# Chanuk-Yang/Deep_Continuous_Fusion_for_Multi-Sensor_3D_Object_Detection

Hardware: AMD Instinct MI355X
Metric: frames/sec (train step) 100k-pt LiDAR + 1242x375 RGB (higher is better)
Workload: dtype bf16; 1 GPU; cfg2: grid 32x704x800, 100000 pts/frame, 1242x375 RGB, ResNet-18 image stream, K=3 fusion x4 sites, eval-mode BN (reference F4), batch 2/GPU; global_batch=2, parallelism=dp1, loss_sampling=compat, conv_chain=False

## Files before the change

### deep_continuous_fusion_for_multi-sensor_3d_object_detection_amd/csrc/geometry.hip

```cpp
#include <stdlib.h>
#include "dcf_common.h"
#include "proj_pred.h"

namespace {

struct Aff6 { float v[6]; };

constexpr int CP_THREADS = 256;
constexpr int CP_ITEMS = 4;
constexpr int CP_TILE = CP_THREADS * CP_ITEMS;

__device__ __forceinline__ int block_excl_scan(int v, int *total)
{
    __shared__ int wsum[4];
    const int lane = threadIdx.x & 63, wid = threadIdx.x >> 6;
    int inc = v;
#pragma unroll
    for (int o = 1; o < 64; o <<= 1) {
        int t = __shfl_up(inc, o, 64);
        if (lane >= o) inc += t;
    }
    if (lane == 63) wsum[wid] = inc;
    __syncthreads();
    int base = 0, tot = 0;
// ... 943 lines not shown
                const int t = t0 + lane;
                int a = 0, b = 0;
                if (R > 0) {
                    if (t < 2 * R + 1) { a = -R; b = -R + t; }
                    else if (t < 4 * R + 2) { a = R; b = -R + (t - (2 * R + 1)); }
                    else if (t < 6 * R + 1) { b = -R; a = -R + 1 + (t - (4 * R + 2)); }
                    else { b = R; a = -R + 1 + (t - (6 * R + 1)); }
                }
                const int bi = I + a, bj = J + b;
                int ps = 0, pe = 0;
                if (t < nblk && bi >= 0 && bi < g.h8 && bj >= 0 && bj < g.w8) {
                    const int k0 = (bi * g.w8 + bj) << 6;
                    ps = cellstart[k0];
                    pe = cellstart[k0 + 64];
                }
                unsigned long long live = __ballot(pe > ps);
                while (live) {
                    const int l = __ffsll((long long)live) - 1;
                    live &= live - 1;
                    const int cbi = __builtin_amdgcn_readlane(bi, l), cbj = __builtin_amdgcn_readlane(bj, l);
                    const int cps = __builtin_amdgcn_readlane(ps, l), cpe = __builtin_amdgcn_readlane(pe, l);
                    bool visit = true;
                    if (gcnt >= K) {
                        const float lox = ((float)(cbi * 8) * s - g.xo) / g.xs, hix = ((float)(cbi * 8 + 8) * s - g.xo) / g.xs;
                        const float loy = ((float)(cbj * 8) * s - g.yo) / g.ys, hiy = ((float)(cbj * 8 + 8) * s - g.yo) / g.ys;
                        const float ddx = fmaxf(0.f, fmaxf(lox - X, X - hix) - 1e-3f);
                        const float ddy = fmaxf(0.f, fmaxf(loy - Y, Y - hiy) - 1e-3f);
                        visit = (ddx * ddx + ddy * ddy) <= gd[K - 1];
                    }
                    if (visit) scan_range(cps, cpe);
                }
            }
            wave_merge<K>(top, gd, gi, gcnt);
            const float bound = (8.0f * (float)R + 0.5f) * cwmin - 1e-3f;
            if (gcnt >= K && gd[K - 1] < bound * bound) done = true;
            if (rmax2 >= 0.0f && bound > 0.f && bound * bound > rmax2) done = true;
        }
    }
    if (lane == 0) {
#pragma unroll
        for (int q = 0; q < K; ++q) out[q * hw + pix] = (q < gcnt) ? gi[q] : -1;
    }
}

template <int K>
__global__ void __launch_bounds__(256) k_knn_search_wave(const int *count, int n_max, KnnGrid g, const int *cellstart,
                                                         const float4 *sorted, float rmax2, int *out)
{
    knn_search_wave<K>(count, n_max, g, cellstart, sorted, rmax2, out, blockIdx.x);
}

constexpr int KNN_FINE_MIN_POINTS = 192;

__device__ __forceinline__ float open_edge_distance(const KnnGrid &gf, float X, float Y, int i0, int i1, int j0, int j1)
{
    const float s = (float)gf.stride;
    float b = 3.0e38f;
    if (i0 > 0) b = fminf(b, X - ((float)i0 * s - gf.xo) / gf.xs);
    if (i1 < gf.h - 1) b = fminf(b, ((float)(i1 + 1) * s - gf.xo) / gf.xs - X);
    if (j0 > 0) b = fminf(b, Y - ((float)j0 * s - gf.yo) / gf.ys);
    if (j1 < gf.w - 1) b = fminf(b, ((float)(j1 + 1) * s - gf.yo) / gf.ys - Y);
    return b - 1e-3f;
}

template <int K>
__device__ __forceinline__ void knn_search_fine(const int *count, int n_max, const KnnGrid &g, const KnnGrid &gf, const int *cellstart_c,
                                                const float4 *sorted_c, const int *cellstart, const float4 *sorted, float rmax2,
                                                int *out, int dense_min, const int bx)
{
    count += blockIdx.y * g.fs_cnt; out += (size_t)blockIdx.y * g.fs_out;
    cellstart_c += (size_t)blockIdx.y * g.fs_ws;
    sorted_c = reinterpret_cast<const float4 *>(reinterpret_cast<const int *>(sorted_c) + (size_t)blockIdx.y * g.fs_ws);
    cellstart += (size_t)blockIdx.y * gf.fs_ws;
    sorted = reinterpret_cast<const float4 *>(reinterpret_cast<const int *>(sorted) + (size_t)blockIdx.y * gf.fs_ws);
    const int lane = threadIdx.x & 63;
    const int pix = __builtin_amdgcn_readfirstlane(bx * 4 + (threadIdx.x >> 6));
    const int hw = g.h * g.w;
    if (pix >= hw) return;
    const int i = pix / g.w, j = pix - i * g.w;
    const float s = (float)g.stride;
    const float X = __fdiv_rn(__fsub_rn(__fmul_rn((float)i + 0.5f, s), g.xo), g.xs);
    const float Y = __fdiv_rn(__fsub_rn(__fmul_rn((float)j + 0.5f, s), g.yo), g.ys);
    const int n = min(*count, n_max);
    int ci, cj;
    point_cell(X, Y, gf, ci, cj);

    TopK<K> top;
    top.clear();
    float gd[K];
    int gi[K];
    int gcnt = 0;
#pragma unroll
    for (int q = 0; q < K; ++q) { gd[q] = 3.0e38f; gi[q] = 0x7fffffff; }
    auto scan_own = [&](int b, int e) {
        for (int p = b; p < e; ++p) {
            const float4 q = sorted[p];
            const float dx = __fsub_rn(q.x, X), dy = __fsub_rn(q.y, Y);
            const float d2 = __fadd_rn(__fmul_rn(dx, dx), __fmul_rn(dy, dy));
            if (!(rmax2 >= 0.0f && d2 > rmax2)) top.insert(d2, __float_as_int(q.z));
        }
    };
    auto scan_range = [&](int b, int e) {
        for (int p = b + lane; p < e; p += 64) {
            const float4 q = sorted_c[p];
            const float dx = __fsub_rn(q.x, X), dy = __fsub_rn(q.y, Y);
            const float d2 = __fadd_rn(__fmul_rn(dx, dx), __fmul_rn(dy, dy));
            if (!(rmax2 >= 0.0f && d2 > rmax2)) top.insert(d2, __float_as_int(q.z));
        }
    };
    bool done = (n == 0);
    bool dense = false;
    if (!done) {
        const int H8 = g.h8 * 8, W8 = g.w8 * 8;
        const int row = lane >> 1, part = lane & 1;
        const int wi = i - 2 + row;
        const int cbeg = max(j - 2, 0), cend = min(j + 2, W8 - 1);
        const int split = min(cend, (cbeg | 7));
        const int c0 = part == 0 ? cbeg : split + 1;
        const int c1 = part == 0 ? split : cend;
        int ps = 0, pe = 0;
        if (lane < 10 && wi >= 0 && wi <= H8 - 1 && c0 <= c1) {
            ps = cellstart_c[cell_key(wi, c0, g)];
            pe = cellstart_c[cell_key(wi, c1, g) + 1];
        }
        const int total = wave_sum_i(pe - ps);
        dense = total > dense_min;
        if (!dense) {
            unsigned long long live = __ballot(pe > ps);
            while (live) {
                const int l = __ffsll((long long)live) - 1;
                live &= live - 1;
                scan_range(__builtin_amdgcn_readlane(ps, l), __builtin_amdgcn_readlane(pe, l));
            }
            wave_merge<K>(top, gd, gi, gcnt);
            const float cw = fminf(s / g.xs, s / g.ys);
            const float bound = 2.5f * cw - 1e-3f;
            if (gcnt >= K && gd[K - 1] < bound * bound) done = true;
            if (rmax2 >= 0.0f && bound > 0.f && bound * bound > rmax2) done = true;
        }
    }
    int rprev = -1;
    for (int r = 2; r <= 8 && !done && dense; r += 2) {
        const int side = 2 * r + 1, ncell = side * side;
        for (int t0 = 0; t0 < ncell; t0 += 64) {
            const int t = t0 + lane;
            const int a = t / side - r, b = t - (t / side) * side - r;
            const int fi = ci + a, fj = cj + b;
            if (t < ncell && max(abs(a), abs(b)) > rprev && fi >= 0 && fi < gf.h && fj >= 0 && fj < gf.w) {
                const int key = cell_key(fi, fj, gf);
                scan_own(cellstart[key], cellstart[key + 1]);
            }
        }
        rprev = r;
        wave_merge<K>(top, gd, gi, gcnt);
        const float bound = open_edge_distance(gf, X, Y, ci - r, ci + r, cj - r, cj + r);
        if (gcnt >= K && bound > 0.f && gd[K - 1] < bound * bound) done = true;
        if (rmax2 >= 0.0f && bound > 0.f && bound * bound > rmax2) done = true;
    }
    if (!done) {
        top.clear();
        gcnt = 0;
#pragma unroll
        for (int q = 0; q < K; ++q) { gd[q] = 3.0e38f; gi[q] = 0x7fffffff; }
        const float cwmin = fminf(s / g.xs, s / g.ys);
        const int I = i >> 3, J = j >> 3;
        const int Rmax = max(g.h8, g.w8);
        for (int R = 0; R <= Rmax && !done; ++R) {
            const int nblk = R == 0 ? 1 : 8 * R;
            for (int t0 = 0; t0 < nblk; t0 += 64) {
                const int t = t0 + lane;
                int a = 0, b = 0;
                if (R > 0) {
                    if (t < 2 * R + 1) { a = -R; b = -R + t; }
                    else if (t < 4 * R + 2) { a = R; b = -R + (t - (2 * R + 1)); }
                    else if (t < 6 * R + 1) { b = -R; a = -R + 1 + (t - (4 * R + 2)); }
                    else { b = R; a = -R + 1 + (t - (6 * R + 1)); }
                }
                const int bi = I + a, bj = J + b;
                int ps = 0, pe = 0;
                if (t < nblk && bi >= 0 && bi < g.h8 && bj >= 0 && bj < g.w8) {
                    const int k0 = (bi * g.w8 + bj) << 6;
                    ps = cellstart_c[k0];
                    pe = cellstart_c[k0 + 64];
                }
                unsigned long long live = __ballot(pe > ps);
                while (live) {
                    const int l = __ffsll((long long)live) - 1;
                    live &= live - 1;
                    const int cbi = __builtin_amdgcn_readlane(bi, l), cbj = __builtin_amdgcn_readlane(bj, l);
                    const int cps = __builtin_amdgcn_readlane(ps, l), cpe = __builtin_amdgcn_readlane(pe, l);
                    bool visit = true;
                    if (gcnt >= K) {
                        const float lox = ((float)(cbi * 8) * s - g.xo) / g.xs, hix = ((float)(cbi * 8 + 8) * s - g.xo) / g.xs;
                        const float loy = ((float)(cbj * 8) * s - g.yo) / g.ys, hiy = ((float)(cbj * 8 + 8) * s - g.yo) / g.ys;
                        const float ddx = fmaxf(0.f, fmaxf(lox - X, X - hix) - 1e-3f);
                        const float ddy = fmaxf(0.f, fmaxf(loy - Y, Y - hiy) - 1e-3f);
                        visit = (ddx * ddx + ddy * ddy) <= gd[K - 1];
                    }
                    if (visit) scan_range(cps, cpe);
                }
            }
            wave_merge<K>(top, gd, gi, gcnt);
            const float bound = (8.0f * (float)R + 0.5f) * cwmin - 1e-3f;
            if (gcnt >= K && gd[K - 1] < bound * bound) done = true;
            if (rmax2 >= 0.0f && bound > 0.f && bound * bound > rmax2) done = true;
        }
    }
    if (lane == 0) {
#pragma unroll
        for (int q = 0; q < K; ++q) out[q * hw + pix] = (q < gcnt) ? gi[q] : -1;
    }
}

template <int K>
__global__ void __launch_bounds__(256) k_knn_search_fine(const int *count, int n_max, KnnGrid g, KnnGrid gf, const int *cellstart_c,
                                                         const float4 *sorted_c, const int *cellstart, const float4 *sorted, float rmax2,
                                                         int *out, int dense_min)
{
    knn_search_fine<K>(count, n_max, g, gf, cellstart_c, sorted_c, cellstart, sorted, rmax2, out, dense_min, blockIdx.x);
}

struct KnnSearchSites {
    KnnGrid g[DCF_MAX_KNN_SITES], gf[DCF_MAX_KNN_SITES];
    const int *cellstart[DCF_MAX_KNN_SITES], *cellstart_f[DCF_MAX_KNN_SITES];
    const float4 *sorted[DCF_MAX_KNN_SITES], *sorted_f[DCF_MAX_KNN_SITES];
    int *out[DCF_MAX_KNN_SITES];
    int kind[DCF_MAX_KNN_SITES];
    int first[DCF_MAX_KNN_SITES + 1];
    int n, dense_min;
};

template <int K>
__global__ void __launch_bounds__(256) k_knn_search_ms(const int *count, int n_max, KnnSearchSites S, float rmax2)
{
    int i = 0;
#pragma unroll
    for (int k = 1; k < DCF_MAX_KNN_SITES; ++k) i += (k < S.n && (int)blockIdx.x >= S.first[k]);
    const int lb = (int)blockIdx.x - S.first[i];
    const int wave = __builtin_amdgcn_readfirstlane(threadIdx.x >> 6);
    const KnnGrid &g = S.g[i];
    const int kind = S.kind[i];
    if (kind == 0) {
        const int tile = lb * 4 + wave;
        if (tile >= g.h8 * g.w8) return;
        knn_search_tile<K, 1>(count, n_max, g, S.cellstart[i], S.sorted[i], rmax2, S.out[i], tile, 0);
    } else if (kind == 1) {
        knn_search_tile<K, 4>(count, n_max, g, S.cellstart[i], S.sorted[i], rmax2, S.out[i], lb, wave);
    } else if (kind == 2) {
        knn_search_wave<K>(count, n_max, g, S.cellstart[i], S.sorted[i], rmax2, S.out[i], lb);
    } else {
        knn_search_fine<K>(count, n_max, g, S.gf[i], S.cellstart[i], S.sorted[i], S.cellstart_f[i], S.sorted_f[i], rmax2, S.out[i], S.dense_min, lb);
    }
}

struct InvMaps {
    const int *idx[DCF_MAX_KNN_MAPS];
    int first[DCF_MAX_KNN_MAPS + 1];
    int hw[DCF_MAX_KNN_MAPS], w[DCF_MAX_KNN_MAPS];
    int n;
};

__device__ __forceinline__ int inv_map_of(const InvMaps &m, int e)
{
    int g = 0;
#pragma unroll
    for (int i = 1; i < DCF_MAX_KNN_MAPS; ++i) g += (i < m.n && e >= m.first[i]);
    return g;
}

struct InvRun { int head, len; };
__device__ __forceinline__ InvRun inv_run(int key, int lane)
{
    const int prev = __shfl_up(key, 1, 64);
    const unsigned long long heads = __ballot(lane == 0 || key != prev);
    const unsigned long long below = heads & ((2ull << lane) - 1ull);
    InvRun r;
    r.head = 63 - __clzll(below);
    const unsigned long long above = lane == 63 ? 0ull : (heads >> (lane + 1));
    r.len = (above ? lane + 1 + (__ffsll((long long)above) - 1) : 64) - r.head;
    return r;
}

__global__ void __launch_bounds__(256) k_zero_rows(int *p, int n, int64_t stride)
{
    int4 *row = reinterpret_cast<int4 *>(p + blockIdx.y * stride);
    const int n4 = n >> 2;
    for (int i = blockIdx.x * blockDim.x + threadIdx.x; i < n4; i += gridDim.x * blockDim.x) row[i] = make_int4(0, 0, 0, 0);
    if (blockIdx.x == 0 && threadIdx.x < (n & 3)) p[blockIdx.y * stride + (n4 << 2) + threadIdx.x] = 0;
}

__device__ __forceinline__ int inv_load(const InvMaps &m, int e, int &g)
{
    const int e0 = blockIdx.x * blockDim.x;
    const int gA = __builtin_amdgcn_readfirstlane(inv_map_of(m, e0));
    const int gB = __builtin_amdgcn_readfirstlane(inv_map_of(m, min(e0 + (int)blockDim.x, m.first[m.n]) - 1));
    if (gA == gB) {
        g = gA;
        return m.idx[gA][e - m.first[gA]];
    }
    g = inv_map_of(m, e);
    return m.idx[g][e - m.first[g]];
}

__global__ void __launch_bounds__(256) k_inv_hist(InvMaps m, int n_max, int *cnt)
{
    const int e = blockIdx.x * blockDim.x + threadIdx.x;
    const int lane = threadIdx.x & 63;
    int key = -1;
    if (e < m.first[m.n]) {
        int g;
        const int id = inv_load(m, e, g);
        if (id >= 0 && id < n_max) key = g * (n_max + 1) + id;
    }
    const InvRun r = inv_run(key, lane);
    if (key >= 0 && r.head == lane) atomicAdd(&cnt[key], r.len);
}

__global__ void __launch_bounds__(256) k_inv_fill(InvMaps m, int n_max, int *cursor, int *ent_pix, int *ent_pt)
{
    const int e = blockIdx.x * blockDim.x + threadIdx.x;
    const int lane = threadIdx.x & 63;
    int key = -1, g = 0, id = 0;
    if (e < m.first[m.n]) {
        id = inv_load(m, e, g);
        if (id >= 0 && id < n_max) key = g * (n_max + 1) + id;
    }
    const InvRun r = inv_run(key, lane);
    int base = 0;
    if (key >= 0 && r.head == lane) base = atomicAdd(&cursor[key], r.len);
    base = __shfl(base, r.head, 64);
    if (key < 0) return;
    const int pos = base + (lane - r.head);
    const int p = (e - m.first[g]) % m.hw[g];
    ent_pix[pos] = ((p / m.w[g]) << 16) | (p % m.w[g]);
    ent_pt[pos] = id;
}

}

extern "C" size_t dcf_compact_workspace_bytes(int n) { return sizeof(int) * (size_t)(cdiv(n > 0 ? n : 1, CP_TILE) + 8); }

extern "C" int dcf_range_filter(const float *pts, int n, const float *lim, float *out_pts, int32_t *out_src,
                                int32_t *count_dev, void *ws, dcf_stream_t stream)
{
    DCF_REQUIRE(n >= 0 && lim && count_dev && ws, "dcf_range_filter: bad arguments");
    hipStream_t s = S(stream);
    if (n == 0) { DCF_HIP(hipMemsetAsync(count_dev, 0, sizeof(int), s)); return DCF_OK; }
    RangePred p;
    memcpy(p.lim.v, lim, sizeof(p.lim.v));
    int nb = cdiv(n, CP_TILE);
    int *bs = (int *)ws;
    DCF_LAUNCH_B("compact_count", (double)n * 12.0, s, hipLaunchKernelGGL(k_compact_count<RangePred>, dim3(nb), dim3(CP_THREADS), 0, s, pts, n, p, bs));
    DCF_LAUNCH("compact_scan", s, hipLaunchKernelGGL(k_compact_scan, dim3(1), dim3(CP_THREADS), 0, s, bs, nb, count_dev));
    DCF_LAUNCH_B("compact_scatter", (double)n * (12.0 + 16.0), s, hipLaunchKernelGGL((k_compact_scatter<RangePred, false>), dim3(nb), dim3(CP_THREADS), 0, s, pts, n, p, bs,
                                                         (float *)nullptr, out_pts, out_src));
    return DCF_OK;
}

extern "C" int dcf_project_filter(const float *pts, int n, const float *lim, const float *crt, float ulim, float vlim,
                                  int mode, float *uv_out, float *xyz_out, int32_t *src_out, int32_t *count_dev,
                                  void *ws, dcf_stream_t stream)
{
    DCF_REQUIRE(n >= 0 && lim && crt && count_dev && ws && uv_out && xyz_out, "dcf_project_filter: bad arguments");
    hipStream_t s = S(stream);
    if (n == 0) { DCF_HIP(hipMemsetAsync(count_dev, 0, sizeof(int), s)); return DCF_OK; }
    ProjPred p;
    memcpy(p.lim.v, lim, sizeof(p.lim.v));
    memcpy(p.c.v, crt, sizeof(p.c.v));
    p.ulim = ulim; p.vlim = vlim; p.mode = mode;
    int nb = cdiv(n, CP_TILE);
    int *bs = (int *)ws;
    DCF_LAUNCH_B("project_count", (double)n * 12.0, s, hipLaunchKernelGGL(k_compact_count<ProjPred>, dim3(nb), dim3(CP_THREADS), 0, s, pts, n, p, bs));
    DCF_LAUNCH("compact_scan", s, hipLaunchKernelGGL(k_compact_scan, dim3(1), dim3(CP_THREADS), 0, s, bs, nb, count_dev));
    DCF_LAUNCH_B("project_scatter", (double)n * (12.0 + 20.0), s, hipLaunchKernelGGL((k_compact_scatter<ProjPred, true>), dim3(nb), dim3(CP_THREADS), 0, s, pts, n, p, bs,
                                                         uv_out, xyz_out, src_out));
    return DCF_OK;
}

extern "C" int dcf_project_filter_batch(const float *const *pts, const int *n, int B, const float *lim, const float *crt, float ulim, float vlim,
                                        int mode, float *uv_out, float *xyz_out, int rows, int32_t *count_dev, void *ws, dcf_stream_t stream)
{
    const char *who = "dcf_project_filter_batch";
    DCF_REQUIRE(pts && n && lim && crt && count_dev && ws && uv_out && xyz_out, "%s: bad arguments", who);
    DCF_REQUIRE(B >= 1 && B <= DCF_PROJ_BATCH_MAX, "%s: 1..%d frames per call", who, DCF_PROJ_BATCH_MAX);
    hipStream_t s = S(stream);
    ProjBatch pb;
    int nmax = 0;
    for (int b = 0; b < DCF_PROJ_BATCH_MAX; ++b) {
        pb.pts[b] = b < B ? pts[b] : nullptr;
        pb.n[b] = b < B ? n[b] : 0;
        DCF_REQUIRE(b >= B || (n[b] >= 0 && n[b] <= rows && (n[b] == 0 || pts[b])), "%s: frame %d: bad point count / null points", who, b);
        memcpy(pb.c[b].v, crt + 12 * (b < B ? b : 0), sizeof(pb.c[b].v));
        if (b < B && n[b] > nmax) nmax = n[b];
    }
    if (nmax == 0) { DCF_HIP(hipMemsetAsync(count_dev, 0, sizeof(int) * B, s)); return DCF_OK; }
    Lim6 l;
    memcpy(l.v, lim, sizeof(l.v));
    const int nb = cdiv(nmax, CP_TILE);
    const int bstride = (int)(dcf_compact_workspace_bytes(nmax) / sizeof(int));
    int *bs = (int *)ws;
    DCF_LAUNCH_B("project_count", (double)nmax * B * 12.0, s, hipLaunchKernelGGL(k_proj_count_b, dim3(nb, B), dim3(CP_THREADS), 0, s, pb, l, ulim, vlim, mode, bs, bstride));
    DCF_LAUNCH("compact_scan", s, hipLaunchKernelGGL(k_proj_scan_b, dim3(1, B), dim3(CP_THREADS), 0, s, bs, nb, bstride, count_dev));
    DCF_LAUNCH_B("project_scatter", (double)nmax * B * (12.0 + 20.0), s, hipLaunchKernelGGL(k_proj_scatter_b, dim3(nb, B), dim3(CP_THREADS), 0, s, pb, l, ulim, vlim, mode, bs, bstride,
                                                                                    uv_out, xyz_out, rows));
    return DCF_OK;
}

extern "C" int dcf_augment_points_batch(const float *const *pts, const int *n, int B, const float *mat, const uint64_t *drop_key,
                                        const uint32_t *drop_thresh, float *const *out, dcf_stream_t stream)
{
    const char *who = "dcf_augment_points_batch";
    DCF_REQUIRE(pts && n && mat && drop_key && drop_thresh && out, "%s: bad arguments", who);
    DCF_REQUIRE(B >= 1 && B <= DCF_PROJ_BATCH_MAX, "%s: 1..%d frames per call", who, DCF_PROJ_BATCH_MAX);
    AugBatch ab;
    int nmax = 0;
    double total = 0.0;
    for (int b = 0; b < DCF_PROJ_BATCH_MAX; ++b) {
        const bool live = b < B;
        DCF_REQUIRE(!live || (n[b] >= 0 && (n[b] == 0 || (pts[b] && out[b]))), "%s: frame %d: bad point count / null points", who, b);
        DCF_REQUIRE(!live || ((((uintptr_t)pts[b]) | ((uintptr_t)out[b])) & 3) == 0, "%s: frame %d: pointers must be 4-byte aligned", who, b);
        ab.pts[b] = live ? pts[b] : nullptr;
        ab.out[b] = live ? out[b] : nullptr;
        ab.key[b] = live ? drop_key[b] : 0;
        ab.n[b] = live ? n[b] : 0;
        ab.thr[b] = live ? drop_thresh[b] : 0;
        for (int k = 0; k < 5; ++k) ab.m[b][k] = live ? mat[5 * b + k] : 0.f;
        if (live && n[b] > nmax) nmax = n[b];
        if (live) total += n[b];
    }
    for (int b = 0; b < B; ++b)
        for (int c = 0; c < B; ++c) {
            if (!n[b] || !n[c]) continue;
            const uintptr_t o0 = (uintptr_t)out[b], o1 = o0 + 12 * (uintptr_t)n[b];
            const uintptr_t p0 = (uintptr_t)pts[c], p1 = p0 + 12 * (uintptr_t)n[c];
            const uintptr_t q0 = (uintptr_t)out[c], q1 = q0 + 12 * (uintptr_t)n[c];
            DCF_REQUIRE((b == c && o0 == p0) || o1 <= p0 || p1 <= o0, "%s: output of frame %d overlaps the input of frame %d", who, b, c);
            DCF_REQUIRE(b == c || o1 <= q0 || q1 <= o0, "%s: outputs of frames %d and %d overlap", who, b, c);
        }
    if (nmax == 0) return DCF_OK;
    hipStream_t s = S(stream);
    DCF_LAUNCH_B("augment_points", total * 24.0, s, hipLaunchKernelGGL(k_augment_points_b, dim3(cdiv(nmax, AUG_TILE), B), dim3(AUG_THREADS), 0, s, ab));
    return DCF_OK;
}

extern "C" size_t dcf_voxelize_workspace_bytes(int Cz, int L, int W) { return sizeof(int) * 2 * (size_t)Cz * L * W; }

static bool voxel_cells_inside(const float *lim, const float *aff, int Cz, int L, int W, int64_t *lo_flat, int64_t *hi_flat)
{
    int64_t lo[3], hi[3];
    for (int ax = 0; ax < 3; ++ax) {
        const float p0 = nextafterf(lim[2 * ax], INFINITY), p1 = nextafterf(lim[2 * ax + 1], -INFINITY);
        if (!(p0 <= p1)) { *lo_flat = *hi_flat = 0; return true; }
        const float t0 = p0 * aff[2 * ax], t1 = p1 * aff[2 * ax];
        const float f0 = t0 + aff[2 * ax + 1], f1 = t1 + aff[2 * ax + 1];
        if (!(fabsf(f0) < 1073741824.0f && fabsf(f1) < 1073741824.0f)) return false;
        const int64_t c0 = (int64_t)(int)f0, c1 = (int64_t)(int)f1;
        lo[ax] = c0 < c1 ? c0 : c1;
        hi[ax] = c0 < c1 ? c1 : c0;
    }
    *lo_flat = (lo[2] * L + lo[0]) * W + lo[1];
    *hi_flat = (hi[2] * L + hi[0]) * W + hi[1];
    return *lo_flat >= 0 && *hi_flat < (int64_t)Cz * L * W;
}

static int voxel_guard(const char *who, const float *lim, const float *aff, int Cz, int L, int W)
{
    for (int k = 0; k < 6; ++k)
        DCF_REQUIRE(fabsf(lim[k]) <= 3.402823466e38f && fabsf(aff[k]) <= 3.402823466e38f, "%s: lim and aff must be finite", who);
    int64_t lo = 0, hi = 0;
    DCF_REQUIRE(voxel_cells_inside(lim, aff, Cz, L, W, &lo, &hi),
                "%s: a point inside the limits can fall into a cell outside the grid (flat cell index %lld .. %lld of %lld voxels)", who,
                (long long)lo, (long long)hi, (long long)Cz * L * W);
    return DCF_OK;
}


extern "C" int dcf_voxelize(const float *pts, int n, const float *lim, const float *aff, int Cz, int L, int W,
                            int mode, float *grid, void *owner_ws, dcf_stream_t stream)
{
    DCF_REQUIRE(n >= 0 && lim && aff && grid && Cz > 0 && L > 0 && W > 0, "dcf_voxelize: bad arguments");
    DCF_REQUIRE((int64_t)Cz * L * W < (1ll << 31), "dcf_voxelize: grid too large for int32 voxel ids");
    if (int rc = voxel_guard("dcf_voxelize", lim, aff, Cz, L, W)) return rc;
    hipStream_t s = S(stream);
    const int nvox = Cz * L * W;
    DCF_HIP(hipMemsetAsync(grid, 0, sizeof(float) * (size_t)nvox, s));
    if (n == 0) return DCF_OK;
    Lim6 l; Aff6 a;
    memcpy(l.v, lim, sizeof(l.v));
    memcpy(a.v, aff, sizeof(a.v));
    const int nb = cdiv(n, 256);
    if (mode == DCF_VOXEL_COMPAT) {
        DCF_REQUIRE(owner_ws != nullptr, "dcf_voxelize: compat mode needs the zeroed owner workspace");
        VoxBatch vb;
        for (int b = 0; b < DCF_MAX_VOXEL_BATCH; ++b) { vb.pts[b] = b == 0 ? pts : nullptr; vb.n[b] = b == 0 ? n : 0; }
        const dim3 g1(nb, 1);
        DCF_LAUNCH("voxel_cell_claim", s, hipLaunchKernelGGL(k_voxel_cell_claim, g1, dim3(256), 0, s, vb, l, a, L, W, nvox, (int *)owner_ws, 0));
        DCF_LAUNCH("voxel_cell_gather", s, hipLaunchKernelGGL((k_voxel_cell_gather<float, false>), g1, dim3(256), 0, s, vb, l, a, Cz, L, W, nvox, grid, (const int *)owner_ws));
        DCF_LAUNCH("voxel_cell_claim", s, hipLaunchKernelGGL(k_voxel_cell_claim, g1, dim3(256), 0, s, vb, l, a, L, W, nvox, (int *)owner_ws, 1));
    } else if (mode == DCF_VOXEL_COMPAT_ROUNDS) {
        DCF_REQUIRE(owner_ws != nullptr, "dcf_voxelize: compat mode needs the zeroed owner workspace");
        for (int r = 0; r <= 8; ++r)
            DCF_LAUNCH("voxel_compat_round", s, hipLaunchKernelGGL(k_voxel_compat_round, dim3(nb), dim3(256), 0, s, pts, n, l, a, L, W, nvox, r,
                                                                   grid, (int *)owner_ws));
    } else if (mode == DCF_VOXEL_ACCUM) {
        DCF_LAUNCH("voxel_accum", s, hipLaunchKernelGGL(k_voxel_accum, dim3(nb), dim3(256), 0, s, pts, n, l, a, L, W, nvox, grid));
    } else if (mode == DCF_VOXEL_OCCUPANCY) {
        DCF_LAUNCH("voxel_occupancy", s, hipLaunchKernelGGL(k_voxel_occupancy, dim3(nb), dim3(256), 0, s, pts, n, l, a, L, W, nvox, grid));
    } else {
        dcf_set_error("dcf_voxelize: unknown mode %d", mode);
        return DCF_EINVAL;
    }
    return DCF_OK;
}

static int voxelize_batch_impl(const char *who, int dtype, bool nhwc, const float *const *pts, const int *n, int B, const float *lim, const float *aff,
                               int Cz, int L, int W, void *grids, void *owner_ws, hipStream_t s)
{
    DCF_REQUIRE(pts && n && lim && aff && grids && owner_ws && Cz > 0 && L > 0 && W > 0, "%s: bad arguments", who);
    DCF_REQUIRE(B >= 1 && B <= DCF_MAX_VOXEL_BATCH, "%s: 1..%d frames per call", who, DCF_MAX_VOXEL_BATCH);
    DCF_REQUIRE((int64_t)Cz * L * W < (1ll << 31), "%s: grid too large for int32 voxel ids", who);
    if (int rc = voxel_guard(who, lim, aff, Cz, L, W)) return rc;
    const int nvox = Cz * L * W;
    const size_t es = dtype == DCF_F32 ? 4 : 2;
    DCF_HIP(hipMemsetAsync(grids, 0, es * (size_t)nvox * B, s));
    VoxBatch vb;
    int nmax = 0;
    for (int b = 0; b < DCF_MAX_VOXEL_BATCH; ++b) {
        vb.pts[b] = b < B ? pts[b] : nullptr;
        vb.n[b] = b < B ? n[b] : 0;
        DCF_REQUIRE(b >= B || (n[b] >= 0 && (n[b] == 0 || pts[b])), "%s: frame %d: null points", who, b);
        if (b < B && n[b] > nmax) nmax = n[b];
    }
    if (nmax == 0) return DCF_OK;
    Lim6 l; Aff6 a;
    memcpy(l.v, lim, sizeof(l.v));
    memcpy(a.v, aff, sizeof(a.v));
    const dim3 grid(cdiv(nmax, 256), B);
    DCF_LAUNCH_B("voxel_cell_claim", (double)nmax * B * 16.0, s, hipLaunchKernelGGL(k_voxel_cell_claim, grid, dim3(256), 0, s, vb, l, a, L, W, nvox, (int *)owner_ws, 0));
    if (!nhwc) {
        DCF_LAUNCH_B("voxel_cell_gather", (double)nmax * B * (12.0 + 27 * 4.0 + 8 * 4.0), s, hipLaunchKernelGGL((k_voxel_cell_gather<float, false>), grid, dim3(256), 0, s, vb, l, a, Cz, L, W, nvox, (float *)grids, (const int *)owner_ws));
    } else {
        DCF_DISPATCH_DTYPE(dtype, { DCF_LAUNCH_B("voxel_cell_gather", (double)nmax * B * (12.0 + 27 * 4.0 + 8.0 * sizeof(T)), s, hipLaunchKernelGGL((k_voxel_cell_gather<T, true>), grid, dim3(256), 0, s, vb, l, a, Cz, L, W, nvox, (T *)grids, (const int *)owner_ws)); })
    }
    DCF_LAUNCH_B("voxel_cell_claim", (double)nmax * B * 16.0, s, hipLaunchKernelGGL(k_voxel_cell_claim, grid, dim3(256), 0, s, vb, l, a, L, W, nvox, (int *)owner_ws, 1));
    return DCF_OK;
}

extern "C" int dcf_voxelize_batch(const float *const *pts, const int *n, int B, const float *lim, const float *aff, int Cz, int L, int W,
                                  float *grids, void *owner_ws, dcf_stream_t stream)
{
    return voxelize_batch_impl("dcf_voxelize_batch", DCF_F32, false, pts, n, B, lim, aff, Cz, L, W, grids, owner_ws, S(stream));
}

extern "C" int dcf_voxelize_batch_nhwc(int dtype, const float *const *pts, const int *n, int B, const float *lim, const float *aff, int Cz, int L,
                                       int W, void *x_nhwc, void *owner_ws, dcf_stream_t stream)
{
    DCF_REQUIRE(dtype == DCF_F32 || dtype == DCF_BF16 || dtype == DCF_F16, "dcf_voxelize_batch_nhwc: unsupported dtype %d", dtype);
    return voxelize_batch_impl("dcf_voxelize_batch_nhwc", dtype, true, pts, n, B, lim, aff, Cz, L, W, x_nhwc, owner_ws, S(stream));
}

static inline void knn_dims(int h, int w, int &h8, int &w8, int &ncell) { h8 = (h + 7) / 8; w8 = (w + 7) / 8; ncell = h8 * w8 * 64; }

extern "C" size_t dcf_knn_workspace_bytes(int n_max, int h, int w)
{
    int h8, w8, ncell;
    knn_dims(h, w, h8, w8, ncell);
    size_t ints = 3 * (size_t)(ncell + 1) + (size_t)cdiv(ncell + 1, CP_TILE) + 8 + (size_t)n_max;
    ints = (ints + 3) & ~(size_t)3;
    return ints * sizeof(int) + sizeof(float4) * (size_t)n_max + 64;
}

struct KnnFine {
    int h, w, stride;
    const void *ws;
    size_t ws_stride_bytes;
};

struct KnnSearchPlan {
    KnnGrid g, gf;
    const int *cellstart, *cellstart_f;
    const float4 *sorted, *sorted_f;
    int kind;
    int tile_waves, dense_min;
};

static KnnSearchPlan knn_search_plan(const KnnGrid &g, int B, int n_max, int K, const int *cellstart, const float4 *sorted, const KnnFine *fine, bool merged)
{
    KnnSearchPlan pl;
    pl.g = g; pl.gf = g; pl.cellstart = cellstart; pl.sorted = sorted; pl.cellstart_f = nullptr; pl.sorted_f = nullptr;
    pl.tile_waves = 1; pl.dense_min = KNN_FINE_MIN_POINTS;
    static DcfOpt force_o("KNN_KERNEL"); const char *force = force_o.str();
    const bool per_wave = force && force[0] == 'w' ? true : (force && force[0] == 't' ? false : (g.h * g.w <= 20000));
    static DcfOpt tw_o("KNN_TILE_WAVES"); const char *tw = tw_o.str();
    pl.tile_waves = tw && (tw[0] == '1' || tw[0] == '2' || tw[0] == '4') ? tw[0] - '0' : (!merged && g.h8 * g.w8 * B <= 1500 ? 4 : 1);
    if (fine) {
        KnnGrid gf = g;
        gf.h = fine->h; gf.w = fine->w; gf.stride = fine->stride;
        int ncf;
        knn_dims(fine->h, fine->w, gf.h8, gf.w8, ncf);
        gf.fs_ws = B > 1 ? (int)(fine->ws_stride_bytes / 4) : 0;
        const int nscf = ncf + 1, nsbf = cdiv(nscf, CP_TILE);
        size_t intsf = 3 * (size_t)nscf + (size_t)nsbf + 8 + (size_t)n_max;
        intsf = (intsf + 3) & ~(size_t)3;
        static DcfOpt dm_o("KNN_FINE_MIN"); const char *dm = dm_o.str();
        pl.gf = gf;
        pl.cellstart_f = (const int *)fine->ws + nscf;
        pl.sorted_f = (const float4 *)((const char *)fine->ws + intsf * sizeof(int));
        pl.dense_min = dm ? atoi(dm) : KNN_FINE_MIN_POINTS;
        pl.kind = 3;
    } else if (per_wave) pl.kind = 2;
    else pl.kind = pl.tile_waves == 4 ? 1 : 0;
    (void)K;
    return pl;
}

static int knn_bev_impl(const char *who, const float *xyz, const int32_t *count_dev, int B, int n_max, int K, int h, int w, int stride,
                        float xs, float xo, float ys, float yo, float rmax2, int32_t *idx_out, void *ws, size_t ws_stride_bytes, hipStream_t s,
                        const KnnFine *fine = nullptr, bool presorted = false, KnnSearchPlan *defer = nullptr)
{
    DCF_REQUIRE(xyz && count_dev && idx_out && ws, "%s: null pointer", who);
    DCF_REQUIRE(K >= 1 && K <= 8, "%s: K must be 1..8 (got %d)", who, K);
    DCF_REQUIRE(h > 0 && w > 0 && stride > 0 && n_max >= 0 && B >= 1 && B <= 65535, "%s: bad dims", who);
    DCF_REQUIRE(B == 1 || (ws_stride_bytes % 16 == 0 && ws_stride_bytes >= dcf_knn_workspace_bytes(n_max, h, w) && ws_stride_bytes / 4 < (1ull << 31)),
                "%s: workspace stride must be a multiple of 16 bytes and hold one frame's workspace", who);
    KnnGrid g;
    g.h = h; g.w = w; g.stride = stride; g.xs = xs; g.xo = xo; g.ys = ys; g.yo = yo;
    g.fs_xyz = B > 1 ? n_max * 3 : 0; g.fs_cnt = B > 1 ? 1 : 0; g.fs_ws = B > 1 ? (int)(ws_stride_bytes / 4) : 0; g.fs_out = B > 1 ? K * h * w : 0;
    int ncell;
    knn_dims(h, w, g.h8, g.w8, ncell);
    const int nscan = ncell + 1;
    const int nsb = cdiv(nscan, CP_TILE);
    int *cellcnt = (int *)ws;
    int *cellstart = cellcnt + nscan;
    int *cursor = cellstart + nscan;
    int *blocksum = cursor + nscan;
    int *pkey = blocksum + nsb + 8;
    size_t ints = 3 * (size_t)nscan + (size_t)nsb + 8 + (size_t)n_max;
    ints = (ints + 3) & ~(size_t)3;
    float4 *sorted = (float4 *)((char *)ws + ints * sizeof(int));
    const double fB = (double)B;
    if (!presorted) {
        if (B == 1) DCF_HIP(hipMemsetAsync(cellcnt, 0, sizeof(int) * (size_t)nscan, s));
        else if ((ws_stride_bytes & 15) == 0 && ((uintptr_t)cellcnt & 15) == 0)
            DCF_LAUNCH_B("knn_zero", (double)B * nscan * 4.0, s, hipLaunchKernelGGL(k_zero_rows, dim3(std::min(cdiv(nscan, 1024), 256), B), dim3(256), 0, s, cellcnt, nscan, (int64_t)(ws_stride_bytes / 4)));
        else DCF_HIP(hipMemset2DAsync(cellcnt, ws_stride_bytes, 0, sizeof(int) * (size_t)nscan, B, s));
        if (n_max > 0) {
            const int nb = cdiv(n_max, 256);
            DCF_LAUNCH_B("knn_hist", fB * n_max * 16.0, s, hipLaunchKernelGGL(k_knn_hist, dim3(nb, B), dim3(256), 0, s, xyz, count_dev, n_max, g, cellcnt, pkey));
        }
        int *total = blocksum + nsb;
        DCF_LAUNCH("scan_blocksum", s, hipLaunchKernelGGL(k_scan_blocksum, dim3(nsb, B), dim3(CP_THREADS), 0, s, cellcnt, nscan, blocksum, g.fs_ws));
        DCF_LAUNCH("compact_scan", s, hipLaunchKernelGGL(k_compact_scan, dim3(1, B), dim3(CP_THREADS), 0, s, blocksum, nsb, total, g.fs_ws));
        DCF_LAUNCH("scan_apply", s, hipLaunchKernelGGL(k_scan_apply, dim3(nsb, B), dim3(CP_THREADS), 0, s, cellcnt, nscan, blocksum, cellstart, cursor, g.fs_ws));
        if (n_max > 0) {
            const int nb = cdiv(n_max, 256);
            DCF_LAUNCH_B("knn_fill", fB * n_max * (12.0 + 4.0 + 16.0), s, hipLaunchKernelGGL(k_knn_fill, dim3(nb, B), dim3(256), 0, s, xyz, count_dev, n_max, pkey, cursor, sorted, g.fs_xyz, g.fs_cnt, g.fs_ws));
        }
    }
    const KnnSearchPlan pl = knn_search_plan(g, B, n_max, K, cellstart, sorted, fine, defer != nullptr);
    if (defer) { *defer = pl; return DCF_OK; }
    const int nbp = g.h8 * g.w8;
    const int nbw = cdiv(h * w, 4);
    if (pl.kind == 3) {
#define KNN_FCASE(KK)                                                                                                                       \
    case KK:                                                                                                                                \
        DCF_LAUNCH_B("knn_search_fine", fB * ((double)h * w * K * 4.0 + (double)n_max * 16.0), s,                                           \
                     hipLaunchKernelGGL(k_knn_search_fine<KK>, dim3(nbw, B), dim3(256), 0, s, count_dev, n_max, g, pl.gf, cellstart, sorted,   \
                                        pl.cellstart_f, pl.sorted_f, rmax2, idx_out, pl.dense_min));                                        \
        break;
        switch (K) {
            KNN_FCASE(1) KNN_FCASE(2) KNN_FCASE(3) KNN_FCASE(4) KNN_FCASE(5) KNN_FCASE(6) KNN_FCASE(7) KNN_FCASE(8)
        }
#undef KNN_FCASE
        return DCF_OK;
    }
#define KNN_CASE(KK)                                                                                                     \
    case KK:                                                                                                             \
        if (pl.kind == 2)                                                                                                \
            DCF_LAUNCH_B("knn_search_wave", fB * ((double)h * w * K * 4.0 + (double)n_max * 16.0), s, hipLaunchKernelGGL(k_knn_search_wave<KK>, dim3(nbw, B), dim3(256), 0, s, count_dev, n_max, g, \
                                                                cellstart, sorted, rmax2, idx_out));                     \
        else if (pl.tile_waves == 4)                                                                                     \
            DCF_LAUNCH_B("knn_search", fB * ((double)h * w * K * 4.0 + (double)n_max * 16.0), s, hipLaunchKernelGGL((k_knn_search<KK, 4>), dim3(nbp, B), dim3(256), 0, s, count_dev, n_max, g, \
                                                           cellstart, sorted, rmax2, idx_out));                          \
        else if (pl.tile_waves == 2)                                                                                     \
            DCF_LAUNCH_B("knn_search", fB * ((double)h * w * K * 4.0 + (double)n_max * 16.0), s, hipLaunchKernelGGL((k_knn_search<KK, 2>), dim3(nbp, B), dim3(128), 0, s, count_dev, n_max, g, \
                                                           cellstart, sorted, rmax2, idx_out));                          \
        else                                                                                                             \
            DCF_LAUNCH_B("knn_search", fB * ((double)h * w * K * 4.0 + (double)n_max * 16.0), s, hipLaunchKernelGGL((k_knn_search<KK, 1>), dim3(nbp, B), dim3(64), 0, s, count_dev, n_max, g, \
                                                           cellstart, sorted, rmax2, idx_out));                          \
        break;
    switch (K) {
        KNN_CASE(1) KNN_CASE(2) KNN_CASE(3) KNN_CASE(4) KNN_CASE(5) KNN_CASE(6) KNN_CASE(7) KNN_CASE(8)
    }
#undef KNN_CASE
    return DCF_OK;
}

extern "C" int dcf_knn_bev(const float *xyz, const int32_t *count_dev, int n_max, int K, int h, int w, int stride,
                           float xs, float xo, float ys, float yo, float rmax2, int32_t *idx_out, void *ws,
                           dcf_stream_t stream)
{
    return knn_bev_impl("dcf_knn_bev", xyz, count_dev, 1, n_max, K, h, w, stride, xs, xo, ys, yo, rmax2, idx_out, ws, 0, S(stream));
}

extern "C" int dcf_knn_bev_batch(const float *xyz, const int32_t *count_dev, int B, int n_max, int K, int h, int w, int stride,
                                 float xs, float xo, float ys, float yo, float rmax2, int32_t *idx_out, void *ws, size_t ws_stride_bytes,
                                 dcf_stream_t stream)
{
    return knn_bev_impl("dcf_knn_bev_batch", xyz, count_dev, B, n_max, K, h, w, stride, xs, xo, ys, yo, rmax2, idx_out, ws, ws_stride_bytes, S(stream));
}

extern "C" int dcf_knn_bev_batch_shared(const float *xyz, const int32_t *count_dev, int B, int n_max, int K, int h, int w, int stride,
                                        int fine_h, int fine_w, int fine_stride, float xs, float xo, float ys, float yo, float rmax2,
                                        int32_t *idx_out, void *ws, size_t ws_stride_bytes, const void *ws_fine, size_t ws_fine_stride_bytes,
                                        dcf_stream_t stream)
{
    const char *who = "dcf_knn_bev_batch_shared";
    DCF_REQUIRE(ws_fine && fine_h > 0 && fine_w > 0 && fine_stride > 0, "%s: bad fine-site arguments", who);
    DCF_REQUIRE(stride % fine_stride == 0 && h * stride <= fine_h * fine_stride && w * stride <= fine_w * fine_stride,
                "%s: the coarse site must lie on the fine site's grid", who);
    DCF_REQUIRE(B == 1 || (ws_fine_stride_bytes % 16 == 0 && ws_fine_stride_bytes >= dcf_knn_workspace_bytes(n_max, fine_h, fine_w) &&
                           ws_fine_stride_bytes / 4 < (1ull << 31)), "%s: fine workspace stride must be that of the fine site's call", who);
    const KnnFine fine = {fine_h, fine_w, fine_stride, ws_fine, ws_fine_stride_bytes};
    return knn_bev_impl(who, xyz, count_dev, B, n_max, K, h, w, stride, xs, xo, ys, yo, rmax2, idx_out, ws, ws_stride_bytes, S(stream), &fine);
}

extern "C" int dcf_knn_bev_sites(const float *xyz, const int32_t *count_dev, int B, int n_max, int K, const dcf_knn_site *sites, int nsites,
                                 float xs, float xo, float ys, float yo, float rmax2, dcf_stream_t stream)
{
    const char *who = "dcf_knn_bev_sites";
    DCF_REQUIRE(xyz && count_dev && sites && nsites >= 1 && nsites <= DCF_MAX_KNN_SITES, "%s: 1..%d sites", who, DCF_MAX_KNN_SITES);
    DCF_REQUIRE(K >= 1 && K <= 8 && n_max >= 0 && B >= 1 && B * nsites <= 65535, "%s: bad dims", who);
    hipStream_t s = S(stream);
    KnnSortSites ss;
    ss.n = nsites; ss.B = B;
    int max_nsb = 1, max_nscan = 1;
    for (int i = 0; i < DCF_MAX_KNN_SITES; ++i) {
        const dcf_knn_site &t = sites[i < nsites ? i : 0];
        DCF_REQUIRE(t.idx_out && t.ws && t.h > 0 && t.w > 0 && t.stride > 0, "%s: site %d: bad arguments", who, i);
        DCF_REQUIRE(((uintptr_t)t.ws & 15) == 0 && t.ws_stride_bytes % 16 == 0 && t.ws_stride_bytes >= dcf_knn_workspace_bytes(n_max, t.h, t.w) &&
                    t.ws_stride_bytes / 4 < (1ull << 31), "%s: site %d: workspace must be 16-byte aligned, its stride a multiple of 16 bytes that holds one frame's workspace", who, i);
        DCF_REQUIRE(t.fine < i && t.fine >= -1, "%s: site %d: `fine` must name an earlier site of the call (or -1)", who, i);
        KnnGrid &g = ss.g[i];
        g.h = t.h; g.w = t.w; g.stride = t.stride; g.xs = xs; g.xo = xo; g.ys = ys; g.yo = yo;
        g.fs_xyz = B > 1 ? n_max * 3 : 0; g.fs_cnt = B > 1 ? 1 : 0; g.fs_ws = B > 1 ? (int)(t.ws_stride_bytes / 4) : 0; g.fs_out = B > 1 ? K * t.h * t.w : 0;
        int ncell;
        knn_dims(t.h, t.w, g.h8, g.w8, ncell);
        ss.ws[i] = (int *)t.ws;
        ss.nscan[i] = ncell + 1;
        ss.nsb[i] = cdiv(ncell + 1, CP_TILE);
        ss.pkey_off[i] = 3 * ss.nscan[i] + ss.nsb[i] + 8;
        size_t ints = 3 * (size_t)ss.nscan[i] + (size_t)ss.nsb[i] + 8 + (size_t)n_max;
        ints = (ints + 3) & ~(size_t)3;
        ss.sorted_off[i] = (int)ints;
        if (i < nsites) { max_nsb = std::max(max_nsb, ss.nsb[i]); max_nscan = std::max(max_nscan, ss.nscan[i]); }
    }
    const int gy = nsites * B;
    DCF_LAUNCH_B("knn_zero", (double)B * max_nscan * 4.0, s, hipLaunchKernelGGL(k_knn_zero_ms, dim3(std::min(cdiv(max_nscan, 1024), 256), gy), dim3(256), 0, s, ss));
    if (n_max > 0)
        DCF_LAUNCH_B("knn_hist", (double)gy * n_max * 16.0, s, hipLaunchKernelGGL(k_knn_hist_ms, dim3(cdiv(n_max, 256), gy), dim3(256), 0, s, xyz, count_dev, n_max, ss));
    DCF_LAUNCH("scan_blocksum", s, hipLaunchKernelGGL(k_scan_blocksum_ms, dim3(max_nsb, gy), dim3(CP_THREADS), 0, s, ss));
    DCF_LAUNCH("compact_scan", s, hipLaunchKernelGGL(k_compact_scan_ms, dim3(1, gy), dim3(CP_THREADS), 0, s, ss));
    DCF_LAUNCH("scan_apply", s, hipLaunchKernelGGL(k_scan_apply_ms, dim3(max_nsb, gy), dim3(CP_THREADS), 0, s, ss));
    if (n_max > 0)
        DCF_LAUNCH_B("knn_fill", (double)gy * n_max * (12.0 + 4.0 + 16.0), s, hipLaunchKernelGGL(k_knn_fill_ms, dim3(cdiv(n_max, 256), gy), dim3(256), 0, s, xyz, count_dev, n_max, ss));
    static DcfOpt ms_o("KNN_MERGED_SEARCH"); const char *ms = ms_o.str();
    const bool merged = !(ms && ms[0] == '0');
    KnnSearchSites S;
    S.n = nsites; S.dense_min = KNN_FINE_MIN_POINTS;
    int blocks = 0;
    double bytes = 0.0;
    for (int i = 0; i < nsites; ++i) {
        const dcf_knn_site &t = sites[i];
        KnnFine fine;
        if (t.fine >= 0) {
            const dcf_knn_site &f = sites[t.fine];
            DCF_REQUIRE(t.stride % f.stride == 0 && t.h * t.stride <= f.h * f.stride && t.w * t.stride <= f.w * f.stride,
                        "%s: site %d must lie on the grid of its fine site", who, i);
            fine = {f.h, f.w, f.stride, f.ws, f.ws_stride_bytes};
        }
        KnnSearchPlan pl;
        int rc = knn_bev_impl(who, xyz, count_dev, B, n_max, K, t.h, t.w, t.stride, xs, xo, ys, yo, rmax2, t.idx_out, t.ws, t.ws_stride_bytes, s,
                              t.fine >= 0 ? &fine : nullptr, true, merged ? &pl : nullptr);
        if (rc) return rc;
        if (!merged) continue;
        S.g[i] = pl.g; S.gf[i] = pl.gf; S.cellstart[i] = pl.cellstart; S.sorted[i] = pl.sorted; S.cellstart_f[i] = pl.cellstart_f;
        S.sorted_f[i] = pl.sorted_f; S.out[i] = t.idx_out; S.kind[i] = pl.kind; S.dense_min = pl.dense_min;
        S.first[i] = blocks;
        const int tiles = pl.g.h8 * pl.g.w8;
        blocks += pl.kind == 0 ? cdiv(tiles, 4) : (pl.kind == 1 ? tiles : cdiv(t.h * t.w, 4));
        bytes += (double)B * ((double)t.h * t.w * K * 4.0 + (double)n_max * 16.0);
    }
    if (!merged) return DCF_OK;
    for (int i = nsites; i < DCF_MAX_KNN_SITES; ++i) {
        S.g[i] = S.g[0]; S.gf[i] = S.gf[0]; S.cellstart[i] = S.cellstart[0]; S.sorted[i] = S.sorted[0]; S.cellstart_f[i] = S.cellstart_f[0];
        S.sorted_f[i] = S.sorted_f[0]; S.out[i] = S.out[0]; S.kind[i] = S.kind[0];
    }
    for (int i = nsites; i <= DCF_MAX_KNN_SITES; ++i) S.first[i] = blocks;
#define KNN_MCASE(KK)                                                                                                                  \
    case KK:                                                                                                                           \
        DCF_LAUNCH_B("knn_search_sites", bytes, s, hipLaunchKernelGGL(k_knn_search_ms<KK>, dim3(blocks, B), dim3(256), 0, s, count_dev, n_max, S, rmax2)); \
        break;
    switch (K) {
        KNN_MCASE(1) KNN_MCASE(2) KNN_MCASE(3) KNN_MCASE(4) KNN_MCASE(5) KNN_MCASE(6) KNN_MCASE(7) KNN_MCASE(8)
    }
#undef KNN_MCASE
    return DCF_OK;
}

extern "C" size_t dcf_fusion_invert_workspace_bytes(int n_max, int nmaps)
{
    const size_t nscan = (size_t)nmaps * (n_max + 1);
    return sizeof(int) * (2 * nscan + (size_t)cdiv(nscan, CP_TILE) + 8);
}

extern "C" int dcf_fusion_invert(const dcf_knn_map *maps, int nmaps, int K, int n_max, int32_t *start, int32_t *ent_pix, int32_t *ent_pt,
                                 void *ws, dcf_stream_t stream)
{
    DCF_REQUIRE(maps && start && ent_pix && ent_pt && ws && K >= 1 && n_max >= 1, "dcf_fusion_invert: bad arguments");
    DCF_REQUIRE(nmaps >= 1 && nmaps <= DCF_MAX_KNN_MAPS, "dcf_fusion_invert: 1..%d maps per call", DCF_MAX_KNN_MAPS);
    InvMaps m;
    m.n = nmaps;
    int64_t tot = 0;
    for (int i = 0; i < DCF_MAX_KNN_MAPS; ++i) {
        m.idx[i] = nullptr; m.hw[i] = 1; m.w[i] = 1; m.first[i] = (int)tot;
        if (i < nmaps) {
            DCF_REQUIRE(maps[i].idx && maps[i].h >= 1 && maps[i].w >= 1 && maps[i].h < 65536 && maps[i].w < 65536,
                        "dcf_fusion_invert: map %d: null or pixel coordinates beyond 16 bits", i);
            m.idx[i] = maps[i].idx; m.hw[i] = maps[i].h * maps[i].w; m.w[i] = maps[i].w;
            tot += (int64_t)K * m.hw[i];
        }
    }
    m.first[DCF_MAX_KNN_MAPS] = (int)tot;
    for (int i = nmaps; i <= DCF_MAX_KNN_MAPS; ++i) m.first[i] = (int)tot;
    DCF_REQUIRE(tot < (1ll << 31), "dcf_fusion_invert: too many pairs");
    hipStream_t s = S(stream);
    const int total = (int)tot, nscan = nmaps * (n_max + 1), nsb = cdiv(nscan, CP_TILE);
    int *cnt = (int *)ws, *cursor = cnt + nscan, *blocksum = cursor + nscan, *totp = blocksum + nsb;
    DCF_HIP(hipMemsetAsync(cnt, 0, sizeof(int) * (size_t)nscan, s));
    DCF_LAUNCH_B("inv_hist", (double)total * 4.0, s, hipLaunchKernelGGL(k_inv_hist, dim3(cdiv(total, 256)), dim3(256), 0, s, m, n_max, cnt));
    DCF_LAUNCH("scan_blocksum", s, hipLaunchKernelGGL(k_scan_blocksum, dim3(nsb), dim3(CP_THREADS), 0, s, cnt, nscan, blocksum));
    DCF_LAUNCH("compact_scan", s, hipLaunchKernelGGL(k_compact_scan, dim3(1), dim3(CP_THREADS), 0, s, blocksum, nsb, totp));
    DCF_LAUNCH("scan_apply", s, hipLaunchKernelGGL(k_scan_apply, dim3(nsb), dim3(CP_THREADS), 0, s, cnt, nscan, blocksum, start, cursor));
    DCF_LAUNCH_B("inv_fill", (double)total * 12.0, s, hipLaunchKernelGGL(k_inv_fill, dim3(cdiv(total, 256)), dim3(256), 0, s, m, n_max, cursor, ent_pix, ent_pt));
    return DCF_OK;
}

#ifdef KNN_STAMP
extern "C" int dcf_knn_stamps_read(long long *dst, int *dims)
{
    dims[0] = KNN_STAMP_TILES; dims[1] = 16;
    DCF_HIP(hipMemcpyFromSymbol(dst, HIP_SYMBOL(g_knn_stamps), sizeof(long long) * KNN_STAMP_TILES * 16));
    return DCF_OK;
}
#endif
```

Measured before the change: 391.2 frames/s.

## Aggregate fusion-invert histogram and fill per 2D pixel tile via LDS hash table

Replaces the per-element inverse-map histogram and fill kernels with tile-based versions. Each block covers a 16x16 pixel tile and all K neighbours, deduplicates point ids in a shared-memory open-addressing hash table, and issues one global atomic per distinct id per tile instead of one per wave run. This aims to cut global atomic contention, since neighbouring pixels often share the same nearest points. The cost is extra LDS traffic, more syncthreads and CAS probing. The old path stays reachable through an INV_TILES=0 option.

Measured after the change: 378.6 frames/s. -3.2%, worse.

```diff
diff --git a/deep_continuous_fusion_for_multi-sensor_3d_object_detection_amd/csrc/geometry.hip b/deep_continuous_fusion_for_multi-sensor_3d_object_detection_amd/csrc/geometry.hip
--- a/deep_continuous_fusion_for_multi-sensor_3d_object_detection_amd/csrc/geometry.hip
+++ b/deep_continuous_fusion_for_multi-sensor_3d_object_detection_amd/csrc/geometry.hip
@@ -1269,7 +1269,7 @@
     return m.idx[g][e - m.first[g]];
 }
 
-__global__ void __launch_bounds__(256) k_inv_hist(InvMaps m, int n_max, int *cnt)
+__global__ void __launch_bounds__(256) k_inv_hist_runs(InvMaps m, int n_max, int *cnt)
 {
     const int e = blockIdx.x * blockDim.x + threadIdx.x;
     const int lane = threadIdx.x & 63;
@@ -1283,7 +1283,7 @@
     if (key >= 0 && r.head == lane) atomicAdd(&cnt[key], r.len);
 }
 
-__global__ void __launch_bounds__(256) k_inv_fill(InvMaps m, int n_max, int *cursor, int *ent_pix, int *ent_pt)
+__global__ void __launch_bounds__(256) k_inv_fill_runs(InvMaps m, int n_max, int *cursor, int *ent_pix, int *ent_pt)
 {
     const int e = blockIdx.x * blockDim.x + threadIdx.x;
     const int lane = threadIdx.x & 63;
@@ -1301,6 +1301,102 @@
     const int p = (e - m.first[g]) % m.hw[g];
     ent_pix[pos] = ((p / m.w[g]) << 16) | (p % m.w[g]);
     ent_pt[pos] = id;
+}
+
+constexpr int INV_TWL = 4, INV_THL = 8 - INV_TWL;
+constexpr int INV_KPASS = 8;
+constexpr int INV_CAPL_MAX = 12;
+static_assert(2 * 256 * INV_KPASS <= (1 << INV_CAPL_MAX), "the table must stay half empty");
+struct InvTiles {
+    const int *idx[DCF_MAX_KNN_MAPS];
+    int tfirst[DCF_MAX_KNN_MAPS + 1];
+    int h[DCF_MAX_KNN_MAPS], w[DCF_MAX_KNN_MAPS];
+    int n;
+};
+
+__device__ __forceinline__ int inv_tab_insert(int *keys, int *val, int capl, int id, int lane)
+{
+    const InvRun r = inv_run(id, lane);
+    int e = 0, base = 0;
+    if (id >= 0 && r.head == lane) {
+        e = (int)(((unsigned)id * 0x9E3779B1u) >> (32 - capl));
+        for (;;) {
+            const int prev = atomicCAS(&keys[e], -1, id);
+            if (prev == -1 || prev == id) break;
+            e = (e + 1) & ((1 << capl) - 1);
+        }
+        base = atomicAdd(&val[e], r.len);
+    }
+    e = __shfl(e, r.head, 64);
+    base = __shfl(base, r.head, 64);
+    return id < 0 ? -1 : (e | ((base + lane - r.head) << INV_CAPL_MAX));
+}
+
+template <bool FILL>
+__device__ __forceinline__ void inv_tile(const InvTiles &m, int K, int n_max, int capl, int *acc, int *ent_pix, int *ent_pt)
+{
+    extern __shared__ __attribute__((aligned(16))) int inv_tab[];
+    int *keys = inv_tab, *val = inv_tab + (1 << capl);
+    int g = 0;
+#pragma unroll
+    for (int i = 1; i < DCF_MAX_KNN_MAPS; ++i) g += (i < m.n && (int)blockIdx.x >= m.tfirst[i]);
+    const int h = m.h[g], w = m.w[g], hw = h * w, tile = (int)blockIdx.x - m.tfirst[g];
+    const int tpr = (w + (1 << INV_TWL) - 1) >> INV_TWL, ti = tile / tpr, tj = tile - ti * tpr;
+    const int i = (ti << INV_THL) + ((int)threadIdx.x >> INV_TWL), j = (tj << INV_TWL) + ((int)threadIdx.x & ((1 << INV_TWL) - 1));
+    const bool in = i < h && j < w;
+    const int *idx = m.idx[g] + (in ? i * w + j : 0);
+    const int lane = threadIdx.x & 63;
+    acc += g * (n_max + 1);
+    for (int k0 = 0; k0 < K; k0 += INV_KPASS) {
+        if (k0) __syncthreads();
+        for (int t = threadIdx.x; t < (1 << capl); t += 256) { keys[t] = -1; val[t] = 0; }
+        int id[INV_KPASS], slot[INV_KPASS];
+#pragma unroll
+        for (int kk = 0; kk < INV_KPASS; ++kk) {
+            id[kk] = -1;
+            if (in && k0 + kk < K) {
+                const int v = idx[(k0 + kk) * hw];
+                if (v >= 0 && v < n_max) id[kk] = v;
+            }
+        }
+        __syncthreads();
+#pragma unroll
+        for (int kk = 0; kk < INV_KPASS; ++kk) slot[kk] = k0 + kk < K ? inv_tab_insert(keys, val, capl, id[kk], lane) : -1;
+        __syncthreads();
+        int c[INV_KPASS];
+#pragma unroll
+        for (int kk = 0; kk < INV_KPASS; ++kk) c[kk] = (unsigned)slot[kk] < (1u << INV_CAPL_MAX) ? val[slot[kk]] : 0;
+        if (!FILL) {
+#pragma unroll
+            for (int kk = 0; kk < INV_KPASS; ++kk)
+                if (c[kk]) atomicAdd(&acc[id[kk]], c[kk]);
+            continue;
+        }
+#pragma unroll
+        for (int kk = 0; kk < INV_KPASS; ++kk)
+            if (c[kk]) c[kk] = atomicAdd(&acc[id[kk]], c[kk]);
+#pragma unroll
+        for (int kk = 0; kk < INV_KPASS; ++kk)
+            if ((unsigned)slot[kk] < (1u << INV_CAPL_MAX)) val[slot[kk]] = c[kk];
+        __syncthreads();
+#pragma unroll
+        for (int kk = 0; kk < INV_KPASS; ++kk)
+            if (slot[kk] >= 0) {
+                const int pos = val[slot[kk] & ((1 << INV_CAPL_MAX) - 1)] + (slot[kk] >> INV_CAPL_MAX);
+                ent_pix[pos] = (i << 16) | j;
+                ent_pt[pos] = id[kk];
+            }
+    }
+}
+
+__global__ void __launch_bounds__(256) k_inv_hist(InvTiles m, int K, int n_max, int capl, int *cnt)
+{
+    inv_tile<false>(m, K, n_max, capl, cnt, nullptr, nullptr);
+}
+
+__global__ void __launch_bounds__(256) k_inv_fill(InvTiles m, int K, int n_max, int capl, int *cursor, int *ent_pix, int *ent_pt)
+{
+    inv_tile<true>(m, K, n_max, capl, cursor, ent_pix, ent_pt);
 }
 
 }
@@ -1786,30 +1882,42 @@
 {
     DCF_REQUIRE(maps && start && ent_pix && ent_pt && ws && K >= 1 && n_max >= 1, "dcf_fusion_invert: bad arguments");
     DCF_REQUIRE(nmaps >= 1 && nmaps <= DCF_MAX_KNN_MAPS, "dcf_fusion_invert: 1..%d maps per call", DCF_MAX_KNN_MAPS);
+    static DcfOpt tiles_o("INV_TILES"); const char *tiles_e = tiles_o.str();
+    const bool tiles = !(tiles_e && !strcmp(tiles_e, "0"));
     InvMaps m;
-    m.n = nmaps;
-    int64_t tot = 0;
+    InvTiles t;
+    m.n = t.n = nmaps;
+    int64_t tot = 0, ntiles = 0;
     for (int i = 0; i < DCF_MAX_KNN_MAPS; ++i) {
-        m.idx[i] = nullptr; m.hw[i] = 1; m.w[i] = 1; m.first[i] = (int)tot;
+        m.idx[i] = t.idx[i] = nullptr; m.hw[i] = m.w[i] = t.h[i] = t.w[i] = 1; m.first[i] = (int)tot; t.tfirst[i] = (int)ntiles;
         if (i < nmaps) {
             DCF_REQUIRE(maps[i].idx && maps[i].h >= 1 && maps[i].w >= 1 && maps[i].h < 65536 && maps[i].w < 65536,
                         "dcf_fusion_invert: map %d: null or pixel coordinates beyond 16 bits", i);
-            m.idx[i] = maps[i].idx; m.hw[i] = maps[i].h * maps[i].w; m.w[i] = maps[i].w;
+            m.idx[i] = t.idx[i] = maps[i].idx; m.hw[i] = maps[i].h * maps[i].w; m.w[i] = t.w[i] = maps[i].w; t.h[i] = maps[i].h;
             tot += (int64_t)K * m.hw[i];
-        }
-    }
-    m.first[DCF_MAX_KNN_MAPS] = (int)tot;
-    for (int i = nmaps; i <= DCF_MAX_KNN_MAPS; ++i) m.first[i] = (int)tot;
+            ntiles += (int64_t)cdiv(maps[i].h, 1 << INV_THL) * cdiv(maps[i].w, 1 << INV_TWL);
+        }
+    }
+    m.first[DCF_MAX_KNN_MAPS] = (int)tot; t.tfirst[DCF_MAX_KNN_MAPS] = (int)ntiles;
     DCF_REQUIRE(tot < (1ll << 31), "dcf_fusion_invert: too many pairs");
     hipStream_t s = S(stream);
     const int total = (int)tot, nscan = nmaps * (n_max + 1), nsb = cdiv(nscan, CP_TILE);
     int *cnt = (int *)ws, *cursor = cnt + nscan, *blocksum = cursor + nscan, *totp = blocksum + nsb;
+    int capl = 9;
+    while ((1 << capl) < 2 * 256 * (K < INV_KPASS ? K : INV_KPASS)) ++capl;
+    const size_t lds = sizeof(int) * 2 * ((size_t)1 << capl);
     DCF_HIP(hipMemsetAsync(cnt, 0, sizeof(int) * (size_t)nscan, s));
-    DCF_LAUNCH_B("inv_hist", (double)total * 4.0, s, hipLaunchKernelGGL(k_inv_hist, dim3(cdiv(total, 256)), dim3(256), 0, s, m, n_max, cnt));
+    if (tiles)
+        DCF_LAUNCH_B("inv_hist", (double)total * 4.0, s, hipLaunchKernelGGL(k_inv_hist, dim3((int)ntiles), dim3(256), lds, s, t, K, n_max, capl, cnt));
+    else
+        DCF_LAUNCH_B("inv_hist", (double)total * 4.0, s, hipLaunchKernelGGL(k_inv_hist_runs, dim3(cdiv(total, 256)), dim3(256), 0, s, m, n_max, cnt));
     DCF_LAUNCH("scan_blocksum", s, hipLaunchKernelGGL(k_scan_blocksum, dim3(nsb), dim3(CP_THREADS), 0, s, cnt, nscan, blocksum));
     DCF_LAUNCH("compact_scan", s, hipLaunchKernelGGL(k_compact_scan, dim3(1), dim3(CP_THREADS), 0, s, blocksum, nsb, totp));
     DCF_LAUNCH("scan_apply", s, hipLaunchKernelGGL(k_scan_apply, dim3(nsb), dim3(CP_THREADS), 0, s, cnt, nscan, blocksum, start, cursor));
-    DCF_LAUNCH_B("inv_fill", (double)total * 12.0, s, hipLaunchKernelGGL(k_inv_fill, dim3(cdiv(total, 256)), dim3(256), 0, s, m, n_max, cursor, ent_pix, ent_pt));
+    if (tiles)
+        DCF_LAUNCH_B("inv_fill", (double)total * 12.0, s, hipLaunchKernelGGL(k_inv_fill, dim3((int)ntiles), dim3(256), lds, s, t, K, n_max, capl, cursor, ent_pix, ent_pt));
+    else
+        DCF_LAUNCH_B("inv_fill", (double)total * 12.0, s, hipLaunchKernelGGL(k_inv_fill_runs, dim3(cdiv(total, 256)), dim3(256), 0, s, m, n_max, cursor, ent_pix, ent_pt));
     return DCF_OK;
 }
 
```
